# grailbio/bigslice

Measured on AMD Instinct MI355X. Metric: rows/sec (whole node) Reshuffle+Reduce group-by, higher is better.
Workload: dtype int64; 1 GPU; model=Reshuffle+Reduce group-by-sum (BASELINE config 3), rows_total=125000000, rows_per_gpu=125000000, distinct_keys=1000000, global_batch=125000000, parallelism=dp1, device=cuda:0

## Files before the change

bigslice_amd/csrc/ext.hip:

```cpp

#include <torch/extension.h>

#include <ATen/hip/HIPContext.h>
#include <hip/hip_runtime.h>

#include <vector>

#include "hash_partition.hip"
#include "groupby.hip"
#include "groupby_part.hip"
#include "sort.hip"
#include "radix.hip"
#include "runs.hip"
#include "runs_multi.hip"
#include "vecagg.hip"
#include "strings.hip"
#include "expr.hip"
#include "tokenize.hip"
#include "groupby_multi.hip"
#include "iddict.hip"
#include "bytes_gather.hip"

namespace {

#define HIP_CHECK(expr)                                              \
  do {                                                               \
    hipError_t _e = (expr);                                          \
    TORCH_CHECK(_e == hipSuccess, "HIP error: ",                     \
                hipGetErrorString(_e));                              \
  } while (0)

int32_t dtype_code(const torch::Tensor& t) {
  switch (t.scalar_type()) {
    case torch::kInt8: return DT_I8;
    case torch::kUInt8: return DT_U8;
    case torch::kInt16: return DT_I16;
    case torch::kInt32: return DT_I32;
    case torch::kInt64: return DT_I64;
    case torch::kFloat32: return DT_F32;
    case torch::kFloat64: return DT_F64;
    case torch::kBool: return DT_BOOL;
    case torch::kUInt32: return DT_U32;
    case torch::kUInt64: return DT_U64;
    default:
      TORCH_CHECK(false, "unsupported column dtype ", t.scalar_type());
  }
}

KeyCols make_key_cols(const std::vector<torch::Tensor>& cols) {
  TORCH_CHECK(!cols.empty() && (int)cols.size() <= MAX_KEY_COLS,
              "1..", MAX_KEY_COLS, " key columns supported");
  KeyCols k;
  k.n = (int)cols.size();
  for (size_t i = 0; i < cols.size(); ++i) {
    TORCH_CHECK(cols[i].is_cuda() && cols[i].is_contiguous(),
                "key columns must be contiguous device tensors");
    k.cols[i] = {cols[i].data_ptr(), dtype_code(cols[i])};
  }
  return k;
}

hipStream_t current_stream() {
  return at::hip::getCurrentHIPStream().stream();
}

int grid_blocks(int64_t n, int threads = THREADS) {
  return (int)std::min<int64_t>((n + threads - 1) / threads, 32768);
}

#define LAUNCH_NK(kernel, nk, blocks, threads, ...)                       \
  do {                                                                    \
    switch (nk) {                                                         \
      case 2:                                                             \
        hipLaunchKernelGGL(kernel<2>, dim3(blocks), dim3(threads), 0,     \
                           current_stream(), __VA_ARGS__);                \
        break;                                                            \
      case 3:                                                             \
        hipLaunchKernelGGL(kernel<3>, dim3(blocks), dim3(threads), 0,     \
                           current_stream(), __VA_ARGS__);                \
        break;                                                            \
      case 4:                                                             \
        hipLaunchKernelGGL(kernel<4>, dim3(blocks), dim3(threads), 0,     \
                           current_stream(), __VA_ARGS__);                \
        break;                                                            \
      default:                                                            \
        hipLaunchKernelGGL(kernel<0>, dim3(blocks), dim3(threads), 0,     \
                           current_stream(), __VA_ARGS__);                \
    }                                                                     \
    HIP_CHECK(hipGetLastError());                                         \
  } while (0)

int64_t int64_cols(const std::vector<torch::Tensor>& cols, int lo, int hi,
                   const char* what) {
// ... 351 lines not shown
  HIP_CHECK(hipGetLastError());
  return clean;
}

void groupby_insert_part(torch::Tensor keys, torch::Tensor vals,
                         torch::Tensor tkeys, torch::Tensor tab,
                         torch::Tensor flags, int64_t max_probes,
                         int64_t nbuckets, int64_t owned,
                         int64_t group_tiles) {
  TORCH_CHECK(keys.is_cuda() && keys.scalar_type() == torch::kInt64);
  TORCH_CHECK(vals.scalar_type() == torch::kInt64 &&
              vals.size(0) == keys.size(0));
  TORCH_CHECK(tab.scalar_type() == torch::kInt64);
  keys = keys.contiguous();
  vals = vals.contiguous();
  if (keys.size(0) == 0) return;
  int64_t cap = table_cap(tkeys, {tab}, flags);
  auto parts = part_scatter_impl(keys, vals, cap, nbuckets, group_tiles);
  const torch::Tensor& pairs = std::get<0>(parts);
  if (owned)
    part_owned_impl(pairs, std::get<1>(parts), tkeys, tab, flags,
                    max_probes);
  else
    launch_gbp_aggregate(pairs, tkeys, tab, flags, cap, max_probes);
}

std::tuple<torch::Tensor, torch::Tensor> groupby_part_scatter(
    torch::Tensor keys, torch::Tensor vals, int64_t cap,
    int64_t nbuckets, int64_t group_tiles) {
  TORCH_CHECK(keys.is_cuda() && keys.scalar_type() == torch::kInt64);
  TORCH_CHECK(vals.scalar_type() == torch::kInt64 &&
              vals.size(0) == keys.size(0));
  return part_scatter_impl(keys.contiguous(), vals.contiguous(), cap,
                           nbuckets, group_tiles);
}

void groupby_part_aggregate(torch::Tensor pairs, torch::Tensor tkeys,
                            torch::Tensor tab, torch::Tensor flags,
                            int64_t max_probes) {
  TORCH_CHECK(pairs.is_cuda() && pairs.scalar_type() == torch::kInt64 &&
              pairs.is_contiguous() && pairs.dim() == 2 &&
              pairs.size(1) == 2);
  if (pairs.size(0) == 0) return;
  TORCH_CHECK(tab.scalar_type() == torch::kInt64);
  launch_gbp_aggregate(pairs, tkeys, tab, flags,
                       table_cap(tkeys, {tab}, flags), max_probes);
}

torch::Tensor groupby_part_owned(torch::Tensor pairs, torch::Tensor totals,
                                 torch::Tensor tkeys, torch::Tensor tab,
                                 torch::Tensor flags, int64_t max_probes) {
  TORCH_CHECK(pairs.is_cuda() && pairs.scalar_type() == torch::kInt64 &&
              pairs.is_contiguous() && pairs.dim() == 2 &&
              pairs.size(1) == 2);
  TORCH_CHECK(totals.is_cuda() && totals.scalar_type() == torch::kInt32 &&
              totals.is_contiguous() && totals.dim() == 1);
  TORCH_CHECK(tab.scalar_type() == torch::kInt64);
  return part_owned_impl(pairs, totals, tkeys, tab, flags, max_probes);
}

std::vector<torch::Tensor> groupby_compact(torch::Tensor tkeys,
                                           std::vector<torch::Tensor> tabs,
                                           torch::Tensor cursor) {
  int64_t cap = tkeys.size(0) - 1;
  CompactCols cc;
  cc.n = (int)tabs.size();
  std::vector<torch::Tensor> out;
  auto out_keys = torch::empty({cap}, tkeys.options());
  out.push_back(out_keys);
  for (size_t c = 0; c < tabs.size(); ++c) {
    out.push_back(torch::empty({cap}, tabs[c].options()));
    cc.tab[c] = {tabs[c].data_ptr(), dtype_code(tabs[c])};
    cc.out[c] = {out[c + 1].data_ptr(), dtype_code(tabs[c])};
  }
  int64_t spb = (cap + 2047) / 2048;
  if (spb < THREADS) spb = THREADS;
  int blocks = (int)((cap + spb - 1) / spb);
  hipLaunchKernelGGL(k_groupby_compact, dim3(blocks), dim3(THREADS), 0,
                     current_stream(), tkeys.data_ptr<int64_t>(), cap, spb,
                     cc, out_keys.data_ptr<int64_t>(),
                     (unsigned long long*)cursor.data_ptr());
  HIP_CHECK(hipGetLastError());
  return out;
}


uint64_t gbm_fp_mask(int64_t fp_bits) {
  TORCH_CHECK(fp_bits >= 1 && fp_bits <= 64, "fp_bits must be in [1, 64]");
  return fp_bits == 64 ? ~uint64_t(0) : (uint64_t(1) << fp_bits) - 1;
}

int64_t gbm_batch_keys(MkCols& kc, const std::vector<torch::Tensor>& keys) {
  const int64_t n = int64_cols(keys, 2, MAX_KEY_COLS, "key columns");
  kc.n = (int)keys.size();
  for (size_t c = 0; c < keys.size(); ++c) {
    kc.src[c] = keys[c].data_ptr<int64_t>();
    kc.tab[c] = nullptr;
  }
  return n;
}

int64_t gbm_table(MkCols& kc, const torch::Tensor& tags,
                  const std::vector<torch::Tensor>& kcols,
                  at::ArrayRef<torch::Tensor> tabs,
                  const torch::Tensor& flags) {
  const int64_t cap = table_cap(tags, tabs, flags);
  TORCH_CHECK(cap <= (int64_t(1) << 31), "capacity above 2^31");
  TORCH_CHECK(flags.numel() >= 3, "flags must be int32[3]");
  TORCH_CHECK((int)kcols.size() == kc.n, "one key array per key column");
  for (size_t c = 0; c < kcols.size(); ++c) {
    TORCH_CHECK(kcols[c].is_cuda() && kcols[c].is_contiguous() &&
                kcols[c].scalar_type() == torch::kInt64 &&
                kcols[c].dim() == 1 && kcols[c].size(0) == cap + 1);
    kc.tab[c] = kcols[c].data_ptr<int64_t>();
  }
  return cap;
}

torch::Tensor groupby_mk_fingerprint(std::vector<torch::Tensor> keys,
                                     int64_t fp_bits) {
  MkCols kc{};
  const int64_t n = gbm_batch_keys(kc, keys);
  const uint64_t fp_mask = gbm_fp_mask(fp_bits);
  auto out = torch::empty({n}, keys[0].options());
  if (n == 0) return out;
  LAUNCH_NK(k_gbm_fingerprint, kc.n, grid_blocks(n), THREADS, kc, n,
            GB_HASH_SEED, fp_mask, out.data_ptr<int64_t>());
  return out;
}

torch::Tensor groupby_mk_claim(std::vector<torch::Tensor> keys,
                               torch::Tensor tags,
                               std::vector<torch::Tensor> kcols,
                               torch::Tensor flags, int64_t max_probes,
                               int64_t fp_bits) {
  MkCols kc{};
  const int64_t n = gbm_batch_keys(kc, keys);
  const int64_t cap = gbm_table(kc, tags, kcols, {}, flags);
  const uint64_t fp_mask = gbm_fp_mask(fp_bits);
  TORCH_CHECK(max_probes >= 1);
  auto slots = torch::empty({n}, keys[0].options().dtype(torch::kInt32));
  if (n == 0) return slots;
  LAUNCH_NK(k_gbm_claim, kc.n, grid_blocks(n), THREADS, kc, n,
            tags.data_ptr<int64_t>(), cap, GB_HASH_SEED, fp_mask,
            (uint32_t*)slots.data_ptr<int32_t>(),
            flags.data_ptr<int32_t>() + 1, max_probes);
  return slots;
}

void groupby_mk_accum(std::vector<torch::Tensor> keys,
                      std::vector<torch::Tensor> vals,
                      std::vector<int64_t> aggs, torch::Tensor slots,
                      torch::Tensor tags, std::vector<torch::Tensor> kcols,
                      std::vector<torch::Tensor> tabs,
                      torch::Tensor flags) {
  MkCols kc{};
  const int64_t n = gbm_batch_keys(kc, keys);
  const int64_t cap = gbm_table(kc, tags, kcols, tabs, flags);
  TORCH_CHECK(keys.size() + vals.size() <= (size_t)MAX_COLS,
              "at most ", MAX_COLS, " key and value columns");
  TORCH_CHECK(slots.is_cuda() && slots.is_contiguous() &&
              slots.scalar_type() == torch::kInt32 && slots.dim() == 1 &&
              slots.size(0) == n);
  ValCols vc = make_val_cols(vals, tabs, aggs);
  for (const auto& v : vals)
    TORCH_CHECK(v.dim() == 1 && v.size(0) == n,
// ... 737 lines not shown
                     overflow.data_ptr<int32_t>(), max_probes);
  HIP_CHECK(hipGetLastError());
}


std::vector<torch::Tensor> bytes_gather(torch::Tensor data,
                                        torch::Tensor offsets,
                                        torch::Tensor rows, int64_t total) {
  TORCH_CHECK(data.is_cuda() && data.is_contiguous() && data.dim() == 1 &&
                  data.scalar_type() == torch::kUInt8,
              "bytes_gather: contiguous uint8 device data required");
  TORCH_CHECK(offsets.is_cuda() && offsets.is_contiguous() &&
                  offsets.dim() == 1 && offsets.size(0) >= 1 &&
                  offsets.scalar_type() == torch::kInt64,
              "bytes_gather: contiguous int64 device offsets required");
  TORCH_CHECK(rows.is_cuda() && rows.dim() == 1 &&
                  rows.scalar_type() == torch::kInt64,
              "bytes_gather: int64 device row indices required");
  rows = rows.contiguous();
  const int64_t n = offsets.size(0) - 1;
  const int64_t m = rows.size(0);
  auto out_offsets = torch::zeros({m + 1}, offsets.options());
  if (m == 0 || total == 0)
    return {torch::empty({0}, data.options()), out_offsets};
  auto stream = current_stream();
  auto lens = torch::empty({m}, offsets.options());
  hipLaunchKernelGGL(k_bg_lens, dim3(grid_blocks(m)), dim3(THREADS), 0,
                     stream, offsets.data_ptr<int64_t>(), n,
                     rows.data_ptr<int64_t>(), m, lens.data_ptr<int64_t>());
  HIP_CHECK(hipGetLastError());
  auto incl = out_offsets.narrow(0, 1, m);
  at::cumsum_out(incl, lens, 0);
  if (total < 0) total = out_offsets[m].item<int64_t>();
  if (total == 0) return {torch::empty({0}, data.options()), out_offsets};
  auto out_data = torch::empty({total}, data.options());
  TORCH_CHECK(((uintptr_t)out_data.data_ptr<uint8_t>() & 15) == 0,
              "bytes_gather: output must be 16-byte aligned");
  const int64_t ntiles = (total + BG_TILE - 1) / BG_TILE;
  TORCH_CHECK(ntiles < (int64_t(1) << 31), "bytes_gather: result too large");
  hipLaunchKernelGGL(k_bg_copy, dim3((uint32_t)ntiles), dim3(BG_BLOCK), 0,
                     stream, data.data_ptr<uint8_t>(), data.size(0),
                     offsets.data_ptr<int64_t>(), n,
                     rows.data_ptr<int64_t>(), m,
                     out_offsets.data_ptr<int64_t>(), total,
                     out_data.data_ptr<uint8_t>());
  HIP_CHECK(hipGetLastError());
  return {out_data, out_offsets};
}

}

PYBIND11_MODULE(TORCH_EXTENSION_NAME, m) {
  m.def("hash_columns", &hash_columns, "murmur3 row hash (K3)");
  m.def("hash_partition", &hash_partition,
        "fused hash+histogram+scatter partitioner (K4)");
  m.def("scatter_by_partition", &scatter_by_partition,
        "scatter rows by precomputed partition ids");
  m.def("groupby_insert", &groupby_insert,
        "hash-aggregate insert pass (K9)");
  m.def("groupby_insert_lds", &groupby_insert_lds,
        "two-level LDS+global insert (int64 sum)");
  m.def("groupby_insert_part", &groupby_insert_part,
        "partitioned LDS pre-aggregating insert (single i64 sum)",
        py::arg("keys"), py::arg("vals"), py::arg("tkeys"), py::arg("tab"),
        py::arg("flags"), py::arg("max_probes"), py::arg("nbuckets"),
        py::arg("owned") = 0, py::arg("group_tiles") = 0);
  m.def("groupby_part_owned", &groupby_part_owned,
        "owner + cleanup passes of the partitioned insert; returns clean");
  m.attr("GBP_OWN_LIMIT") = (int64_t)GBP_OWN_LIMIT;
  m.def("groupby_part_scatter", &groupby_part_scatter,
        "bucket scatter of the partitioned insert", py::arg("keys"),
        py::arg("vals"), py::arg("cap"), py::arg("nbuckets"),
        py::arg("group_tiles") = 0);
  m.def("groupby_part_group_tiles", &part_group_tiles,
        "tiles per group the partitioned insert picks for n rows");
  m.attr("GBP_SCATTER_ROWS") = (int64_t)GBP_SCATTER_ROWS;
  m.def("groupby_part_aggregate", &groupby_part_aggregate,
        "aggregate pass of the partitioned insert");
  m.attr("GBP_TILE_ROWS") = (int64_t)GBP_TILE_ROWS;
  m.attr("GBP_LDS_SLOTS") = (int64_t)GBP_LDS_SLOTS;
  m.attr("GBP_MAX_BUCKETS") = (int64_t)GBP_MAX_BUCKETS;
  m.def("groupby_compact", &groupby_compact,
        "hash-aggregate table compaction (K9)");
  m.def("groupby_mk_insert", &groupby_mk_insert,
        "multi-column-key hash-aggregate insert: claim + accumulate (K21)",
        py::arg("keys"), py::arg("vals"), py::arg("aggs"), py::arg("tags"),
        py::arg("kcols"), py::arg("tabs"), py::arg("flags"),
        py::arg("max_probes"), py::arg("fp_bits") = 64);
  m.def("groupby_mk_claim", &groupby_mk_claim,
        "launch 1 of groupby_mk_insert; returns the rows' slots");
  m.def("groupby_mk_accum", &groupby_mk_accum,
        "launch 2 of groupby_mk_insert");
  m.def("groupby_mk_fingerprint", &groupby_mk_fingerprint,
        "the tuple fingerprint groupby_mk_insert claims slots by",
        py::arg("keys"), py::arg("fp_bits") = 64);
  m.attr("MAX_KEY_COLS") = (int64_t)MAX_KEY_COLS;
  m.attr("MAX_COLS") = (int64_t)MAX_COLS;
  m.def("agg_identity", &agg_identity, "aggregation identity fill");
  m.def("radix_argsort", &radix_argsort, "device radix argsort (K6)");
  m.def("radix_sort_keys", &radix_sort_keys, "device radix key sort",
        py::arg("keys"), py::arg("probe") = true);
  m.def("runs_sorted", &runs_sorted,
        "run boundaries of sorted keys (K18)");
  m.def("runs_multi", &runs_multi,
        "run boundaries of lexicographically sorted key columns (K22)");
  m.attr("MRUNS_TILE_ROWS") = (int64_t)MRUNS_TILE;
  m.def("lex_searchsorted", &lex_searchsorted,
        "searchsorted over lexicographically sorted tuples (K22)",
        py::arg("sorted_cols"), py::arg("query_cols"),
        py::arg("right") = false);
  m.def("segment_reduce_runs", &segment_reduce_runs,
        "int64 segmented reduce with precomputed runs (K16 fast path)");
  m.def("runs_guard", &runs_guard,
        "(count, max run length) of a runs_sorted result");
  m.def("segment_reduce_sorted", &segment_reduce_sorted,
        "typed reduce-by-key over sorted pairs (K16; deterministic)");
  m.def("hash_bytes", &hash_bytes,
        "murmur3-32 over varlen byte rows (K17, device strings)");
  m.def("hash_bytes64", &hash_bytes64,
        "64-bit two-seed murmur3 dictionary ids (K17)");
  m.def("colsum16", &colsum16,
        "vector-aggregate experiment: [N,16] f32 colsum, VALU vs MFMA");
  m.def("radix_sort_kv", &radix_sort_kv,
        "direct (key, 8-byte value) radix sort");
  m.def("slot_pids", &slot_pids, "table-slot-range partition ids");
  m.def("expr_apply", &expr_apply,
        "fused Map/Filter expression interpreter (K13)");
  m.def("tokenize_bytes", &tokenize_bytes,
        "split BYTES rows into tokens on a delimiter set (K20)");
  m.attr("TOKENIZE_TILE_BYTES") = (int64_t)TOK_TILE;
  m.def("iddict_claim", &iddict_claim,
        "id dictionary: claim slots for new ids; returns the new rows (K23)");
  m.def("iddict_lookup", &iddict_lookup,
        "id dictionary: position of every id, -1 when absent (K23)");
  m.def("iddict_rehash", &iddict_rehash,
        "id dictionary: move a table into a larger one (K23)");
  m.def("bytes_gather", &bytes_gather,
        "variable-length row gather of a BYTES column (K23)",
        py::arg("data"), py::arg("offsets"), py::arg("rows"),
        py::arg("total") = -1);
  m.attr("BYTES_GATHER_TILE_BYTES") = (int64_t)BG_TILE;
}
```

bigslice_amd/csrc/groupby.hip:

```cpp

#include <hip/hip_runtime.h>

#include "hashtable.h"

#define THREADS 256

struct CompactCols {
  ColDesc tab[MAX_COLS];
  MutColDesc out[MAX_COLS];
  int n;
};

__device__ __forceinline__ void copy_elt(const MutColDesc& dst, int64_t di,
                                         const ColDesc& src, int64_t si) {
  switch (elt_size(src.code)) {
    case 1: ((uint8_t*)dst.ptr)[di] = ((const uint8_t*)src.ptr)[si]; break;
    case 2: ((uint16_t*)dst.ptr)[di] = ((const uint16_t*)src.ptr)[si]; break;
    case 4: ((uint32_t*)dst.ptr)[di] = ((const uint32_t*)src.ptr)[si]; break;
    default: ((uint64_t*)dst.ptr)[di] = ((const uint64_t*)src.ptr)[si];
  }
}

extern "C" __global__ void k_groupby_compact(
    const int64_t* tkeys, int64_t cap, int64_t slots_per_block,
// ... 58 lines not shown
    if (cur == GB_SENTINEL) {
      long long prev = atomicCAS((unsigned long long*)&lk[h],
                                 (unsigned long long)GB_SENTINEL,
                                 (unsigned long long)k);
      cur = (prev == GB_SENTINEL) ? k : prev;
    }
    if (cur == k) {
      atomicAdd((unsigned long long*)&lv[h], (unsigned long long)v);
      return true;
    }
    h = (h + 1) & (GB_LDS_SLOTS - 1);
  }
  return false;
}

extern "C" __global__ void k_groupby_insert_sum_i64_lds(
    const int64_t* keys, const int64_t* vals, int64_t n, int64_t* tkeys,
    long long* tab, int64_t cap, uint32_t seed, int32_t* sentinel_seen,
    int32_t* overflow, int64_t max_probes) {
  __shared__ long long lk[GB_LDS_SLOTS];
  __shared__ long long lv[GB_LDS_SLOTS];
  for (int i = threadIdx.x; i < GB_LDS_SLOTS; i += blockDim.x) {
    lk[i] = GB_SENTINEL;
    lv[i] = 0;
  }
  __syncthreads();
  uint64_t gmask = (uint64_t)cap - 1;
  int64_t stride = (int64_t)gridDim.x * blockDim.x;
  int64_t i = (int64_t)blockIdx.x * blockDim.x + threadIdx.x;
  for (; i < n; i += stride) {
    int64_t k = keys[i];
    long long v = (long long)vals[i];
    if (k == GB_SENTINEL || !gb_lds_try(k, v, lk, lv, seed))
      gb_global_insert_sum(k, v, tkeys, tab, gmask, cap, seed,
                           sentinel_seen, overflow, max_probes);
  }
  __syncthreads();
  for (int i2 = threadIdx.x; i2 < GB_LDS_SLOTS; i2 += blockDim.x) {
    if (lk[i2] != GB_SENTINEL)
      gb_global_insert_sum(lk[i2], lv[i2], tkeys, tab, gmask, cap, seed,
                           sentinel_seen, overflow, max_probes);
  }
}

extern "C" __global__ void k_slot_pids(const int64_t* keys, int64_t n,
                                       int64_t cap, int32_t nparts,
                                       uint32_t seed, int32_t* pids) {
  int64_t i = (int64_t)blockIdx.x * blockDim.x + threadIdx.x;
  int64_t stride = (int64_t)gridDim.x * blockDim.x;
  uint64_t mask = (uint64_t)cap - 1;
  uint64_t shift = 0;
  while (((uint64_t)cap >> shift) > (uint64_t)nparts) ++shift;
  for (; i < n; i += stride) {
    uint64_t h = mm3_u64((uint64_t)keys[i], seed) & mask;
    pids[i] = (int32_t)(h >> shift);
  }
}

extern "C" __global__ void k_groupby_insert(
    const int64_t* keys, int64_t n, ValCols vals, int64_t* tkeys,
    int64_t cap, uint32_t seed, int32_t* sentinel_seen, int32_t* overflow,
    int64_t max_probes) {
  int64_t i = (int64_t)blockIdx.x * blockDim.x + threadIdx.x;
  int64_t stride = (int64_t)gridDim.x * blockDim.x;
  uint64_t mask = (uint64_t)cap - 1;
  for (; i < n; i += stride) {
    int64_t k = keys[i];
    int64_t slot;
    if (k == GB_SENTINEL) {
      if (atomicOr(sentinel_seen, 1) == 0) {}
      slot = cap;
    } else {
      uint64_t h = mm3_u64((uint64_t)k, seed) & mask;
      if (gb_probe_claim(tkeys, h, mask, k, max_probes) == GB_FULL) {
        atomicOr(overflow, 1);
        return;
      }
      slot = (int64_t)h;
    }
    for (int c = 0; c < vals.n; ++c)
      accum(vals.tab[c], slot, vals.src[c], i, vals.agg[c]);
  }
}
```

bigslice_amd/kernels/groupby.py:

```python

from __future__ import annotations

import dataclasses
import math
import os
import sys
from typing import List, Optional

import torch

from .. import kernels as _k
from . import _C, native
from .sortedkeys import sort_combine

_AGG_CODES = {"sum": 0, "min": 1, "max": 2, "prod": 3}

_GB_KEY_DTYPES = (torch.int64,)
_GB_VAL_DTYPES = (torch.int64, torch.int32, torch.float32, torch.float64)

GB_SENTINEL = -(1 << 63)
MAX_PROBES = 128

PART_TILE_ROWS = _C.GBP_TILE_ROWS if _C is not None else None
PART_LDS_SLOTS = _C.GBP_LDS_SLOTS if _C is not None else None
PART_MAX_BUCKETS = _C.GBP_MAX_BUCKETS if _C is not None else None

PART_OWN_LIMIT = _C.GBP_OWN_LIMIT if _C is not None else None


@dataclasses.dataclass(frozen=True)
class Options:
    mode: Optional[str] = None
    combine: str = "auto"
    part: bool = True
    part_owned: bool = True
    part_group: int = 0
    lds_blocks: int = 4096
    sample_rows: int = 1 << 19
    debug: bool = False

    @classmethod
    def from_env(cls, env=None) -> "Options":
        env = os.environ if env is None else env
        mode = env.get("BIGSLICE_GB_MODE")
        return cls(
            mode=mode if mode in ("lds", "global", "part") else None,
            combine=env.get("BIGSLICE_GB_COMBINE", "auto"),
            part=env.get("BIGSLICE_GB_PART", "1") == "1",
            part_owned=env.get("BIGSLICE_GB_PART_OWNED", "1") == "1",
            part_group=int(env.get("BIGSLICE_GB_PART_GROUP", "0")),
            lds_blocks=int(env.get("BIGSLICE_GB_LDS_BLOCKS", "4096")),
            sample_rows=int(env.get("BIGSLICE_GB_SAMPLE_ROWS",
                                    str(1 << 19))),
            debug=bool(env.get("BIGSLICE_GB_DEBUG")))


def _next_pow2(n: int, floor: int = 1024) -> int:
    c = floor
    while c < n:
        c <<= 1
    return c


def first_capacity(cap_hint: Optional[int], n: int, floor: int = 1024) -> int:
    from .. import config
    return _next_pow2(cap_hint or min(
        2 * n, getattr(config, "GROUPBY_INITIAL_CAP", 1 << 23)), floor)


def part_buckets(n: int, nkeys: float, cap: int,
                 lds_slots: int = PART_LDS_SLOTS,
                 tile_rows: int = PART_TILE_ROWS,
                 max_buckets: int = PART_MAX_BUCKETS) -> int:
    room = lds_slots / 2 - tile_rows * nkeys / max(n, 1)
    b = 2
    while b < max_buckets and (room <= 0 or b * room < nkeys):
        b <<= 1
    return min(b, cap)


def part_owned_buckets(n: int, cap: int, lds_slots: int, tile_rows: int,
                       max_buckets: int):
    want = max(cap / lds_slots, n / tile_rows)
    b = 2
    while b < want:
        b <<= 1
    b = max(2, min(b, max_buckets, cap))
    s = cap // b
    return (b, s) if s <= lds_slots else None


PART_BAND = (6.0, 500.0)


def forced_mode(opts: Options, sum_i64: bool) -> Optional[str]:
    if opts.mode in ("lds", "global"):
        return opts.mode
    if opts.mode == "part" and not sum_i64:
        return "global"
    if opts.combine == "sort":
        return "sort"
    return None


def choose_mode(distinct: int, sample_n: int, batch_n: int, sum_i64: bool,
                opts: Options, cap_hint: Optional[int] = None):
    forced = forced_mode(opts, sum_i64)
    if forced:
        return forced, None, cap_hint
    s = sample_n
    K = None
    if distinct < s:
        K = float(distinct)
        for _ in range(20):
            K = distinct / (1.0 - math.exp(-s / K))
        if cap_hint is None:
            cap_hint = _next_pow2(min(max(int(4 * K), 1024), 1 << 30))
    if distinct * 32 <= s:
        mode = "lds"
    elif distinct * 100 > s * 88:
        mode = "sort"
    else:
        rows_per_key = batch_n / max(K, 1.0)
        mode = "sort" if rows_per_key > 500 else "global"
        if (mode == "global" and sum_i64 and opts.part
                and PART_BAND[0] <= rows_per_key <= PART_BAND[1]):
            mode = "part"
    if opts.mode == "part":
        mode = "part"
    elif mode == "sort" and opts.combine == "hash":
        mode = "global"
    return mode, K, cap_hint


def part_plan(n: int, cap: int, key_estimate: Optional[float],
              opts: Options, lds_slots: int, tile_rows: int,
# ... 4 lines not shown
                             max_buckets) if opts.part_owned else None
    if own is not None:
        return "owned", own[0]
    nkeys = key_estimate or cap / 4
    return "tiled", part_buckets(n, nkeys, cap, lds_slots, tile_rows,
                                 max_buckets)


def regrow_capacity(cap: int, rows: int) -> int:
    new = cap
    while new < 4 * rows and new < (1 << 30):
        new <<= 1
    if new == cap:
        new <<= 1
    if new > (1 << 31):
        raise RuntimeError("groupby table overflow")
    return new


def groupby_supported(keys: torch.Tensor, vals: List[torch.Tensor],
                      aggs: List[str]) -> bool:
    return (native(keys.is_cuda, "groupby") and groupby_shape_supported(
        [keys.dtype], [v.dtype for v in vals], aggs))


def groupby_shape_supported(key_dtypes, val_dtypes, aggs) -> bool:
    return (all(dt in _GB_KEY_DTYPES for dt in key_dtypes)
            and all(dt in _GB_VAL_DTYPES for dt in val_dtypes)
            and all(isinstance(a, str) and a in _AGG_CODES for a in aggs))


class HashTable:

    def _ensure_alloc(self, n: int):
        if self.cap is None:
            self._alloc(first_capacity(self.cap_hint, n))

    def _agg_arrays(self, cap: int) -> List:
        return [
            _k._C.agg_identity(torch.empty(0, dtype=dt, device=self.device),
                            code, cap + 1)
            for dt, code in zip(self.val_dtypes, self.codes)]

    def _compact(self):
        cursor = torch.zeros(1, dtype=torch.int64, device=self.device)
        outs = _k._C.groupby_compact(*self._slots(), cursor)
        host = torch.cat([cursor, self.flags.to(torch.int64)]).cpu()
        return outs, host.tolist()

    def _regrow(self):
        batches = self.batches
        self._alloc(regrow_capacity(self.cap, self.rows))
        self.batches = []
        for keys, vals in batches:
            self._insert_now(keys, vals)


class GroupTable(HashTable):

    _SMALL_BATCH = 1 << 21
    _PART_MIN_ROWS = 1 << 21

    def __init__(self, val_dtypes, aggs: List[str], device,
                 cap_hint: int = None):
        self.opts = Options.from_env()
        self.aggs = aggs
        self.codes = [_AGG_CODES[a] for a in aggs]
        self.device = device
        self.val_dtypes = list(val_dtypes)
        self.cap = None
        self.cap_hint = cap_hint
        self.tkeys = None
        self.tabs: List = []
        self.flags = None
        self.batches: List = []
        self._deferred: List = []
        self.rows = 0
        self._mode: Optional[str] = None
        self._sample_forced: Optional[str] = None
        self._sample_n = 0
        self._sample_batch_n = 0
        self._sample_ne = None
        self._key_estimate: Optional[float] = None

    @property
    def _sum_i64(self) -> bool:
        return (len(self.val_dtypes) == 1
                and self.val_dtypes[0] == torch.int64
                and self.aggs == ["sum"])

    def _alloc(self, cap: int):
        self.cap = cap
        dev = self.device
        self.tkeys = torch.full((cap + 1,), GB_SENTINEL,
                                dtype=torch.int64, device=dev)
        self.tabs = self._agg_arrays(cap)
        self.flags = torch.zeros(2, dtype=torch.int32, device=dev)

    def _slots(self):
        return self.tkeys, self.tabs

    @property
    def _sort_combinable(self) -> bool:
        return (_k._C is not None
                and str(self.device).startswith("cuda")
                and all(a in ("sum", "min", "max") for a in self.aggs)
                and all(dt in _GB_VAL_DTYPES for dt in self.val_dtypes))

    def _start_sample(self, keys: torch.Tensor) -> None:
        self._sample_forced = forced_mode(self.opts, self._sum_i64)
        if self._sample_forced:
            return
        prefix = min(keys.shape[0], self.opts.sample_rows)
        sk = _k._C.radix_sort_keys(keys[:prefix].contiguous(),
                                probe=False)
        self._sample_n = prefix
        self._sample_batch_n = keys.shape[0]
        self._sample_ne = (sk[1:] != sk[:-1]).sum()

    def _read_sample(self) -> str:
        if self._sample_forced:
            return self._sample_forced
        distinct = 1 + int(self._sample_ne.item())
        mode, self._key_estimate, self.cap_hint = choose_mode(
            distinct, self._sample_n, self._sample_batch_n, self._sum_i64,
            self.opts, self.cap_hint)
        if self.opts.debug:
            print(f"[gb] sample={self._sample_n} distinct={distinct} "
                  f"cap_hint={self.cap_hint} mode={mode}",
                  file=sys.stderr, flush=True)
        return mode

    def insert(self, keys: torch.Tensor, vals: List[torch.Tensor]):
        n = keys.shape[0]
        if n == 0:
            return
        self.rows += n
        if not self._sort_combinable:
            self._insert_now(keys, vals)
            return
        if self._mode is None:
            if n >= self._SMALL_BATCH:
                self._start_sample(keys)
                self._mode = "pending"
            self._deferred.append((keys, vals))
            return
        if self._mode == "pending":
            self._mode = self._read_sample()
        if self._mode == "sort":
            self._deferred.append((keys, vals))
            return
        self._flush_deferred()
        self._insert_now(keys, vals)

    def _flush_deferred(self):
        pending, self._deferred = self._deferred, []
        for k, v in pending:
            self._insert_now(k, v)

    def _insert_now(self, keys: torch.Tensor, vals: List[torch.Tensor]):
        self._ensure_alloc(keys.shape[0])
        self.batches.append((keys, vals))
        mode = self._mode if self._sum_i64 else None
        plan = part_plan(
            keys.shape[0], self.cap, self._key_estimate, self.opts,
            PART_LDS_SLOTS, PART_TILE_ROWS, PART_MAX_BUCKETS,
            self._PART_MIN_ROWS) if mode == "part" else None
        if mode == "lds":
            _k._C.groupby_insert_lds(keys, vals[0], self.tkeys, self.tabs[0],
                                  self.flags, MAX_PROBES,
                                  self.opts.lds_blocks)
        elif plan is not None:
            kind, nbuckets = plan
            _k._C.groupby_insert_part(keys, vals[0], self.tkeys, self.tabs[0],
                                   self.flags, MAX_PROBES, nbuckets,
                                   1 if kind == "owned" else 0,
                                   self.opts.part_group)
        else:
            _k._C.groupby_insert(keys, list(vals), self.codes, self.tkeys,
                              self.tabs, self.flags, MAX_PROBES)

    def _finish_deferred(self):
        from ..utils import stats
        if self._mode not in (None, "sort"):
            self._flush_deferred()
            return None
        batches = self._deferred
        keys = (batches[0][0] if len(batches) == 1
                else torch.cat([k for k, _ in batches]))
        if self._mode is None:
            self._start_sample(keys)
            self._mode = self._read_sample()
            if self._mode != "sort":
                self._flush_deferred()
                return None
        self._deferred = []
        vcols = (list(batches[0][1]) if len(batches) == 1
                 else [torch.cat(cols)
                       for cols in zip(*(v for _, v in batches))])
        uk, outs = sort_combine(keys, vcols, self.codes)
        if self.cap is not None:
            self._insert_now(uk, outs)
            return None
        stats.DEFAULT.add("combiner/keys", int(uk.shape[0]))
        return uk, outs

    def finish(self):
        from ..utils import stats
        stats.DEFAULT.add("combiner/records", self.rows)
        if self._mode == "pending":
            self._mode = self._read_sample()
        if self._deferred:
            done = self._finish_deferred()
            if done is not None:
                return done
        if self.cap is None:
            empty = torch.empty(0, dtype=torch.int64, device=self.device)
            return empty, [torch.empty(0, dtype=dt, device=self.device)
                           for dt in self.val_dtypes]
        while True:
            outs, (nkeys, sentinel_seen, overflow) = self._compact()
            if overflow:
                self._regrow()
                continue
            keys = outs[0][:nkeys]
            vals = [o[:nkeys] for o in outs[1:]]
            if sentinel_seen:
                keys = torch.cat([keys, torch.full(
                    (1,), GB_SENTINEL, dtype=torch.int64,
                    device=self.device)])
                vals = [torch.cat([v, t[self.cap:self.cap + 1]])
                        for v, t in zip(vals, self.tabs)]
            self.batches = []
            stats.DEFAULT.add("combiner/keys", int(keys.shape[0]))
            return keys, vals


def groupby(keys: torch.Tensor, vals: List[torch.Tensor],
            aggs: List[str]):
    t = GroupTable([v.dtype for v in vals], aggs, keys.device)
    t.insert(keys, list(vals))
    return t.finish()
```

bigslice_amd/ops/aggregate.py:

```python

from __future__ import annotations

import functools
import operator
import os
from typing import Callable, List, Optional, Sequence, Union

import torch

from .. import config
from ..frame import Frame
from ..schema import Schema, is_object

BUILTIN_AGGS = ("sum", "min", "max", "prod")

_CALLABLE_MAP = {
    operator.add: "sum",
    operator.mul: "prod",
    min: "min",
    max: "max",
}


def resolve_agg(fn: Union[str, Callable]) -> Union[str, Callable]:
# ... 188 lines not shown

    def result_frames(self, chunk: int):
        for f in self.inner.result_frames(chunk):
            pos = torch.searchsorted(
                self.dict_ids, f.columns[0].to(self.dict_ids.device))
            keys = self.dict_keys.select(pos)
            yield Frame([keys] + list(f.columns[1:]), 1,
                        combined_id=f.combined_id)


class TensorAggregator:

    def __init__(self, schema: Schema, agg: Aggregation, device: str):
        self.schema = schema
        self.nkey = schema.prefix
        self.agg = agg
        self.device = device
        self.keys: Optional[List[torch.Tensor]] = None
        self.vals: List[torch.Tensor] = []
        self._pending = _Pending()
        self._pt_frames: Optional[List[Frame]] = []
        self._pt_id = None
        self._table = None
        if device.startswith("cuda"):
            from .. import kernels
            from ..kernels import groupby_multi as gbm
            if self.nkey == 1:
                supported = kernels.groupby_shape_supported
                make = kernels.GroupTable
            else:
                def supported(*shape):
                    return (gbm.multikey_supported(*shape)
                            and gbm.Options.from_env().enabled)
                make = functools.partial(
                    gbm.MultiKeyTable, self.nkey,
                    fallback=lambda k, v: _combine_once(k, v, self.agg))
            val_dts = schema.dtypes[self.nkey:]
            if supported(schema.dtypes[:self.nkey], val_dts, agg.aggs) \
                    and kernels.native(True, "groupby"):
                self._table = make(val_dts, agg.aggs, device)

    def add(self, frame: Frame) -> None:
        if len(frame) == 0:
            return
        if frame.device != self.device:
            frame = frame.to(self.device)
        if self._pt_frames is not None:
            cid = frame.combined_id
            if cid is not None and (self._pt_id is None
                                    or cid == self._pt_id):
                self._pt_id = cid
                self._pt_frames.append(frame)
                return
            buffered, self._pt_frames = self._pt_frames, None
            for f in buffered:
                self._add_normal(f)
        self._add_normal(frame)

    def _add_normal(self, frame: Frame) -> None:
        if self._table is not None:
            self._pending.feed(frame, self._table_insert)
            return
        self._pending.add(frame)
        if self._pending.rows >= config.COMBINER_TARGET_KEYS:
            self._flush()

    def _table_insert(self, f: Frame) -> None:
        vals = [c.contiguous() for c in f.columns[self.nkey:]]
        if self.nkey == 1:
            self._table.insert(f.columns[0].contiguous(), vals)
        else:
            self._table.insert(list(f.columns[:self.nkey]), vals)

    def _flush(self) -> None:
        f = self._pending.take()
        if f is None:
            return
        keys = [c for c in f.columns[: self.nkey]]
        vals = list(f.columns[self.nkey:])
        if self.keys is not None:
            keys = [torch.cat([sk, k]) for sk, k in zip(self.keys, keys)]
            vals = [torch.cat([sv, v]) for sv, v in zip(self.vals, vals)]
        self.keys, self.vals = _combine_once(keys, vals, self.agg)

    def result_frames(self, chunk: int):
        if self._pt_frames is not None:
            for f in self._pt_frames:
                yield f
            return
        if self._table is not None:
            self._pending.flush(self._table_insert)
            keys, vals = self._table.finish()
            keys = [keys] if self.nkey == 1 else keys
            if keys[0].shape[0]:
                self.keys, self.vals = keys, vals
        else:
            self._flush()
        if self.keys is None:
            return
        import uuid
        cid = uuid.uuid4().int & ((1 << 63) - 1)
        n = self.keys[0].shape[0]
        for off in range(0, n, chunk):
            stop = min(off + chunk, n)
            yield Frame([k[off:stop] for k in self.keys] +
                        [v[off:stop] for v in self.vals],
                        self.schema.prefix, combined_id=cid)


def _combine_once(keys: List[torch.Tensor], vals: List[torch.Tensor],
                  agg: Aggregation):
    from ..kernels.groupby import _AGG_CODES
    from ..kernels.sortedkeys import _SCATTER_OP
    if len(keys) == 1:
        k = keys[0]
        if k.is_cuda:
            from .. import kernels
            if kernels.groupby_supported(k, vals, agg.aggs):
                uk, ov = kernels.groupby(k, vals, agg.aggs)
                return [uk], ov
        uk, inv = torch.unique(k, return_inverse=True)
        nseg = uk.shape[0]
        uks = [uk]
    else:
        n = keys[0].shape[0]
        perm = torch.arange(n, device=keys[0].device)
        for kc in reversed(keys):
            _, o = torch.sort(kc[perm], stable=True)
            perm = perm[o]
        skeys = [kc[perm] for kc in keys]
        boundary = torch.zeros(n, dtype=torch.bool,
                               device=keys[0].device)
        boundary[0] = True
        for kc in skeys:
            boundary[1:] |= kc[1:] != kc[:-1]
        inv_sorted = boundary.cumsum(0) - 1
        nseg = int(inv_sorted[-1].item()) + 1 if n else 0
        uks = [kc[boundary] for kc in skeys]
        inv = torch.empty(n, dtype=torch.int64, device=keys[0].device)
        inv[perm] = inv_sorted
        vals = list(vals)
    out_vals = []
    for v, a in zip(vals, agg.aggs):
        init = torch.empty(nseg, dtype=v.dtype, device=v.device)
        out = init.scatter_reduce_(
            0, inv, v, reduce=_SCATTER_OP[_AGG_CODES[a]], include_self=False)
        out_vals.append(out)
    return uks, out_vals


class DictAggregator:

    def __init__(self, schema: Schema, agg: Aggregation):
        self.schema = schema
        self.agg = agg
        self.state = {}

    def add(self, frame: Frame) -> None:
        nkey = self.schema.prefix
        lists = frame.column_lists()
        keys = list(zip(*lists[:nkey])) if nkey > 1 else lists[0]
        vals = lists[nkey:]
        state = self.state
        aggs = self.agg.aggs
        if len(vals) == 1 and aggs == ["sum"]:
            vcol = vals[0]
# ... 53 lines not shown
```

bigslice_amd/runtime/partition.py:

```python

from __future__ import annotations

from typing import Callable, List, Optional

import torch

from ..frame import Frame


def partition_ids(frame: Frame, num_partitions: int,
                  partitioner: Optional[Callable] = None) -> torch.Tensor:
    if partitioner is not None:
        p = partitioner(frame, num_partitions)
        if not isinstance(p, torch.Tensor):
            p = torch.tensor(list(p), dtype=torch.int64)
        return p.to(torch.int64)
    h = frame.hash(0)
    return (h.to(torch.int64) & 0xFFFFFFFF) % num_partitions


def split_frame(frame: Frame, num_partitions: int,
                partitioner: Optional[Callable] = None) -> List[Optional[Frame]]:
    if num_partitions == 1:
        return [frame]
    if len(frame) == 0:
        return [None] * num_partitions
    if frame.device != "cpu" and not frame.has_objects:
        from .. import kernels
        if num_partitions <= 4096 and kernels.partition_supported(frame):
            return kernels.partition_frame(frame, num_partitions,
                                           partitioner)
    p = partition_ids(frame, num_partitions, partitioner)
    order = torch.argsort(p, stable=True)
    sorted_f = frame.select(order)
    counts = torch.bincount(p, minlength=num_partitions)
    out: List[Optional[Frame]] = []
    off = 0
    for c in counts.tolist():
        out.append(sorted_f.slice(off, off + c) if c else None)
        off += c
    return out


class SharedPhaseCombiner:

    def __init__(self, schema, combiner, device: str, num_partitions: int,
                 expected_tasks: int, chunk: int):
        import threading

        from ..ops.aggregate import make_aggregator
        self.agg = make_aggregator(schema, combiner, device)
        self.device = device
        self.num_partitions = num_partitions
        self.chunk = chunk
        self.remaining = expected_tasks
        self.lock = threading.Lock()
        self.events = []
        self.rows = 0

    def add(self, frame: Frame) -> None:
        with self.lock:
            self.rows += len(frame)
            self.agg.add(frame)

    def task_done(self) -> bool:
        if self.device.startswith("cuda"):
            ev = torch.cuda.Event()
            ev.record()
        else:
            ev = None
        with self.lock:
            if ev is not None:
                self.events.append(ev)
            self.remaining -= 1
            return self.remaining == 0

    def finish_buckets(self) -> List[List[Frame]]:
        if self.device.startswith("cuda"):
            cur = torch.cuda.current_stream()
            for ev in self.events:
                cur.wait_event(ev)
        buckets: List[List[Frame]] = \
            [[] for _ in range(self.num_partitions)]
        for f in self.agg.result_frames(self.chunk * 4):
            for pi, pf in enumerate(split_frame(f, self.num_partitions,
                                                None)):
                if pf is not None and len(pf):
                    buckets[pi].append(pf)
        return buckets


class PartitionWriter:

    def __init__(self, num_partitions: int, partitioner, combiner,
                 schema, device: str, chunk: int):
        self.num_partitions = num_partitions
        self.partitioner = partitioner
        self.schema = schema
        self.device = device
        self.chunk = chunk
        self.rows = 0
        self.agg = None
        self.aggs = None
        self.buckets: List[List[Frame]] = \
            [[] for _ in range(num_partitions)]
        if combiner is not None:
            from ..ops.aggregate import make_aggregator
            if partitioner is None:
                self.agg = make_aggregator(schema, combiner, device)
            else:
                self.aggs = [make_aggregator(schema, combiner, device)
                             for _ in range(num_partitions)]

    def add(self, frame: Frame) -> None:
        self.rows += len(frame)
        if self.agg is not None:
            self.agg.add(frame)
            return
        parts = split_frame(frame, self.num_partitions, self.partitioner)
        from ..frame import over_high_water
        tier = frame.device != "cpu" and over_high_water()
        for pi, pf in enumerate(parts):
            if pf is None or len(pf) == 0:
                continue
            if self.aggs is not None:
                self.aggs[pi].add(pf)
            elif tier:
                self.buckets[pi].append(pf.to_pinned_host())
            else:
                self.buckets[pi].append(pf)

    def finish(self) -> List[List[Frame]]:
        if self.agg is not None:
            for f in self.agg.result_frames(self.chunk * 4):
                parts = split_frame(f, self.num_partitions, None)
                for pi, pf in enumerate(parts):
                    if pf is not None and len(pf):
                        self.buckets[pi].append(pf)
            return self.buckets
        if self.aggs is not None:
            return [list(a.result_frames(self.chunk)) for a in self.aggs]
        return self.buckets
```

Measured before the change: 29.14 billion rows/sec.

## Compact group-by table directly into hash partitions and hash-sample distinct keys

Adds a three-kernel finish (count, offsets, write) that compacts the hash-aggregate table straight into per-partition contiguous output, so the separate compact followed by split_frame per chunk is no longer needed. It also replaces the sort-based distinct-key sample estimate with a hash-table claim count on the device. Both paths are enabled by default and fall back to the old route when conditions are not met. The cost is an extra histogram pass over the table, plus a host sync for the partition counts.

```diff
diff --git a/bigslice_amd/csrc/ext.hip b/bigslice_amd/csrc/ext.hip
--- a/bigslice_amd/csrc/ext.hip
+++ b/bigslice_amd/csrc/ext.hip
@@ -9,6 +9,7 @@
 #include "hash_partition.hip"
 #include "groupby.hip"
 #include "groupby_part.hip"
+#include "groupby_finish.hip"
 #include "sort.hip"
 #include "radix.hip"
 #include "runs.hip"
@@ -526,6 +527,88 @@
                      (unsigned long long*)cursor.data_ptr());
   HIP_CHECK(hipGetLastError());
   return out;
+}
+
+std::pair<int64_t, int64_t> gbf_blocks(int64_t cap, int64_t nparts) {
+  int64_t blocks = std::min<int64_t>(
+      GBF_THREADS, std::max<int64_t>(64, (int64_t(1) << 18) / nparts));
+  blocks = std::min(blocks, (cap + 1 + 2047) / 2048);
+  int64_t spb = (cap + 1 + blocks - 1) / blocks;
+  spb += spb & 1;
+  return {(cap + 1 + spb - 1) / spb, spb};
+}
+
+std::tuple<std::vector<torch::Tensor>, torch::Tensor>
+groupby_compact_partition(torch::Tensor tkeys,
+                          std::vector<torch::Tensor> tabs,
+                          torch::Tensor flags, int64_t nparts) {
+  TORCH_CHECK(nparts >= 1 && nparts <= MAX_LDS_PARTS &&
+                  nparts <= GBF_MAX_PARTS,
+              "nparts must be in [1, ", MAX_LDS_PARTS, "]");
+  const int64_t cap = table_cap(tkeys, tabs, flags);
+  TORCH_CHECK(cap <= (int64_t(1) << 31), "capacity above 2^31");
+  FinishCols fc;
+  fc.n = (int)tabs.size();
+  TORCH_CHECK(fc.n <= MAX_COLS, "at most ", MAX_COLS, " value columns");
+  std::vector<torch::Tensor> out;
+  out.push_back(torch::empty({cap + 1}, tkeys.options()));
+  for (int c = 0; c < fc.n; ++c) {
+    const auto st = tabs[c].scalar_type();
+    TORCH_CHECK(st == torch::kInt64 || st == torch::kInt32 ||
+                    st == torch::kFloat32 || st == torch::kFloat64,
+                "unsupported value dtype ", st);
+    out.push_back(torch::empty({cap + 1}, tabs[c].options()));
+    fc.tab[c] = {tabs[c].data_ptr(), dtype_code(tabs[c])};
+    fc.out[c] = {out[c + 1].data_ptr(), dtype_code(tabs[c])};
+  }
+  const auto [blocks, spb] = gbf_blocks(cap, nparts);
+  auto opts32 = tkeys.options().dtype(torch::kInt32);
+  auto hist = torch::empty({nparts * blocks}, opts32);
+  auto totals = torch::empty({nparts}, opts32);
+  auto dev = torch::empty({nparts + 2}, tkeys.options());
+  auto stream = current_stream();
+  const uint32_t np = (uint32_t)nparts;
+  const int32_t* fl = flags.data_ptr<int32_t>();
+  hipLaunchKernelGGL(k_gbf_count, dim3((uint32_t)blocks), dim3(GBF_THREADS),
+                     0, stream, tkeys.data_ptr<int64_t>(), cap, spb, np, fl,
+                     (uint32_t*)hist.data_ptr<int32_t>());
+  HIP_CHECK(hipGetLastError());
+  hipLaunchKernelGGL(k_gbf_offsets, dim3(np), dim3(GBF_THREADS), 0, stream,
+                     (uint32_t*)hist.data_ptr<int32_t>(), (uint32_t)blocks,
+                     np, fl, (uint32_t*)totals.data_ptr<int32_t>(),
+                     dev.data_ptr<int64_t>());
+  HIP_CHECK(hipGetLastError());
+  hipLaunchKernelGGL(k_gbf_write, dim3((uint32_t)blocks), dim3(GBF_THREADS),
+                     0, stream, tkeys.data_ptr<int64_t>(), cap, spb, np, fl,
+                     (const uint32_t*)hist.data_ptr<int32_t>(),
+                     (const uint32_t*)totals.data_ptr<int32_t>(), fc,
+                     out[0].data_ptr<int64_t>());
+  HIP_CHECK(hipGetLastError());
+  return {out, dev.cpu()};
+}
+
+torch::Tensor groupby_sample_distinct(torch::Tensor keys, int64_t rows) {
+  TORCH_CHECK(keys.is_cuda() && keys.scalar_type() == torch::kInt64 &&
+              keys.dim() == 1 && keys.stride(0) == 1);
+  TORCH_CHECK(rows >= 1 && rows <= keys.size(0) &&
+                  rows <= (int64_t(1) << 30),
+              "1 <= rows <= min(len(keys), 2^30)");
+  int64_t m = 2;
+  while (m < 2 * rows) m <<= 1;
+  auto tags = torch::empty({m}, keys.options());
+  auto state = torch::empty({2}, keys.options());
+  auto result = state.select(0, 0);
+  auto stream = current_stream();
+  hipLaunchKernelGGL(k_gbs_init, dim3(grid_blocks(m / 2)), dim3(THREADS), 0,
+                     stream, tags.data_ptr<int64_t>(), m,
+                     state.data_ptr<int64_t>());
+  HIP_CHECK(hipGetLastError());
+  hipLaunchKernelGGL(k_gbs_count, dim3(grid_blocks((rows + 1) / 2)),
+                     dim3(THREADS), 0, stream, keys.data_ptr<int64_t>(),
+                     rows, tags.data_ptr<int64_t>(), m,
+                     state.data_ptr<int64_t>());
+  HIP_CHECK(hipGetLastError());
+  return result;
 }
 
 
@@ -1429,6 +1512,11 @@
   m.attr("GBP_MAX_BUCKETS") = (int64_t)GBP_MAX_BUCKETS;
   m.def("groupby_compact", &groupby_compact,
         "hash-aggregate table compaction (K9)");
+  m.def("groupby_compact_partition", &groupby_compact_partition,
+        "compact a group-by table straight into hash partitions");
+  m.attr("MAX_LDS_PARTS") = (int64_t)MAX_LDS_PARTS;
+  m.def("groupby_sample_distinct", &groupby_sample_distinct,
+        "distinct keys of a prefix, minus one, as a device scalar");
   m.def("groupby_mk_insert", &groupby_mk_insert,
         "multi-column-key hash-aggregate insert: claim + accumulate (K21)",
         py::arg("keys"), py::arg("vals"), py::arg("aggs"), py::arg("tags"),
diff --git a/bigslice_amd/csrc/groupby.hip b/bigslice_amd/csrc/groupby.hip
--- a/bigslice_amd/csrc/groupby.hip
+++ b/bigslice_amd/csrc/groupby.hip
@@ -164,3 +164,67 @@
       accum(vals.tab[c], slot, vals.src[c], i, vals.agg[c]);
   }
 }
+
+extern "C" __global__ void k_gbs_init(int64_t* tags, int64_t m,
+                                      int64_t* state) {
+  const int64_t stride = (int64_t)gridDim.x * blockDim.x;
+  int64_t i = (int64_t)blockIdx.x * blockDim.x + threadIdx.x;
+  if (i == 0) {
+    state[0] = -1;
+    state[1] = 0;
+  }
+  const longlong2 empty = {GB_SENTINEL, GB_SENTINEL};
+  for (; 2 * i < m; i += stride) *(longlong2*)(tags + 2 * i) = empty;
+}
+
+__device__ __forceinline__ uint32_t gbs_claim(int64_t k, int64_t* tags,
+                                              uint64_t mask, int32_t* flag) {
+  if (k == GB_SENTINEL)
+    return *(volatile int32_t*)flag == 0 && atomicOr(flag, 1) == 0;
+  uint64_t h = gbm_fmix64((uint64_t)k) & mask;
+  return gb_probe_claim(tags, h, mask, k, (int64_t)mask + 1) == GB_CLAIMED;
+}
+
+template <bool WIDE>
+__device__ __forceinline__ uint32_t gbs_count_rows(const int64_t* keys,
+                                                   int64_t rows,
+                                                   int64_t* tags,
+                                                   uint64_t mask,
+                                                   int32_t* flag) {
+  const int64_t stride = (int64_t)gridDim.x * blockDim.x;
+  int64_t t = (int64_t)blockIdx.x * blockDim.x + threadIdx.x;
+  uint32_t mine = 0;
+  if constexpr (WIDE) {
+    for (int64_t i = 2 * t; i < rows; i += 2 * stride) {
+      if (i + 1 < rows) {
+        const longlong2 two = *(const longlong2*)(keys + i);
+        mine += gbs_claim(two.x, tags, mask, flag);
+        mine += gbs_claim(two.y, tags, mask, flag);
+      } else {
+        mine += gbs_claim(keys[i], tags, mask, flag);
+      }
+    }
+  } else {
+    for (int64_t i = t; i < rows; i += stride)
+      mine += gbs_claim(keys[i], tags, mask, flag);
+  }
+  return mine;
+}
+
+extern "C" __global__ __launch_bounds__(THREADS) void k_gbs_count(
+    const int64_t* keys, int64_t rows, int64_t* tags, int64_t m,
+    int64_t* state) {
+  __shared__ uint32_t claimed;
+  if (threadIdx.x == 0) claimed = 0;
+  __syncthreads();
+  const uint64_t mask = (uint64_t)m - 1;
+  int32_t* flag = (int32_t*)(state + 1);
+  const uint32_t mine =
+      ((uintptr_t)keys & 15) == 0
+          ? gbs_count_rows<true>(keys, rows, tags, mask, flag)
+          : gbs_count_rows<false>(keys, rows, tags, mask, flag);
+  if (mine) atomicAdd(&claimed, mine);
+  __syncthreads();
+  if (threadIdx.x == 0 && claimed)
+    atomicAdd((unsigned long long*)state, (unsigned long long)claimed);
+}
diff --git a/bigslice_amd/csrc/groupby_finish.hip b/bigslice_amd/csrc/groupby_finish.hip
--- /dev/null
+++ b/bigslice_amd/csrc/groupby_finish.hip
@@ -0,0 +1,156 @@
+
+#include <hip/hip_runtime.h>
+
+#include "hashtable.h"
+
+#define GBF_THREADS 512
+#define GBF_WAVES (GBF_THREADS / 64)
+#define GBF_MAX_PARTS 4096
+#define GBF_SCAN_C (GBF_MAX_PARTS / GBF_THREADS)
+
+struct FinishCols {
+  ColDesc tab[MAX_COLS];
+  MutColDesc out[MAX_COLS];
+  int n;
+};
+
+__device__ __forceinline__ uint32_t gbf_part(int64_t k, uint32_t nparts) {
+  return mm3_u64((uint64_t)k, 0u) % nparts;
+}
+
+template <bool WIDE, typename F>
+__device__ __forceinline__ void gbf_live_slots(const int64_t* tkeys,
+                                               int64_t cap, bool sentinel,
+                                               int64_t start, int64_t end,
+                                               F f) {
+  auto one = [&](int64_t i, int64_t k) {
+    if (i < cap ? k != GB_SENTINEL : sentinel) f(i, k);
+  };
+  if constexpr (WIDE) {
+    for (int64_t i = start + 2 * threadIdx.x; i < end;
+         i += 2 * GBF_THREADS) {
+      if (i + 1 < end) {
+        const longlong2 two = *(const longlong2*)(tkeys + i);
+        one(i, two.x);
+        one(i + 1, two.y);
+      } else {
+        one(i, tkeys[i]);
+      }
+    }
+  } else {
+    for (int64_t i = start + threadIdx.x; i < end; i += GBF_THREADS)
+      one(i, tkeys[i]);
+  }
+}
+
+extern "C" __global__ __launch_bounds__(GBF_THREADS) void k_gbf_count(
+    const int64_t* tkeys, int64_t cap, int64_t slots_per_block,
+    uint32_t nparts, const int32_t* flags, uint32_t* hist) {
+  __shared__ uint32_t lh[GBF_MAX_PARTS];
+  for (uint32_t p = threadIdx.x; p < nparts; p += GBF_THREADS) lh[p] = 0;
+  __syncthreads();
+  const int64_t start = (int64_t)blockIdx.x * slots_per_block;
+  const int64_t end = min(start + slots_per_block, cap + 1);
+  const bool sentinel = flags[0] != 0;
+  auto count = [&](int64_t, int64_t k) {
+    atomicAdd(&lh[gbf_part(k, nparts)], 1u);
+  };
+  if (((uintptr_t)tkeys & 15) == 0)
+    gbf_live_slots<true>(tkeys, cap, sentinel, start, end, count);
+  else
+    gbf_live_slots<false>(tkeys, cap, sentinel, start, end, count);
+  __syncthreads();
+  for (uint32_t p = threadIdx.x; p < nparts; p += GBF_THREADS)
+    hist[(int64_t)p * gridDim.x + blockIdx.x] = lh[p];
+}
+
+__device__ __forceinline__ uint32_t gbf_block_scan(uint32_t x,
+                                                   uint32_t* wtmp,
+                                                   uint32_t* total) {
+  const int lane = threadIdx.x & 63;
+  const int w = threadIdx.x >> 6;
+  uint32_t run = x;
+  for (int off = 1; off < 64; off <<= 1) {
+    const uint32_t up = __shfl_up(run, off);
+    if (lane >= off) run += up;
+  }
+  if (lane == 63) wtmp[w] = run;
+  __syncthreads();
+  uint32_t base = 0, all = 0;
+  for (int w2 = 0; w2 < GBF_WAVES; ++w2) {
+    if (w2 < w) base += wtmp[w2];
+    all += wtmp[w2];
+  }
+  *total = all;
+  __syncthreads();
+  return base + run - x;
+}
+
+extern "C" __global__ __launch_bounds__(GBF_THREADS) void k_gbf_offsets(
+    uint32_t* hist, uint32_t nblocks, uint32_t nparts, const int32_t* flags,
+    uint32_t* totals, int64_t* host) {
+  __shared__ uint32_t wtmp[GBF_WAVES];
+  const uint32_t p = blockIdx.x;
+  uint32_t* row = hist + (int64_t)p * nblocks;
+  const bool ok = threadIdx.x < nblocks;
+  const uint32_t x = ok ? row[threadIdx.x] : 0;
+  uint32_t total;
+  const uint32_t excl = gbf_block_scan(x, wtmp, &total);
+  if (ok) row[threadIdx.x] = excl;
+  if (threadIdx.x == 0) {
+    totals[p] = total;
+    host[p] = (int64_t)total;
+    if (p == 0) {
+      host[nparts] = flags[0];
+      host[nparts + 1] = flags[1];
+    }
+  }
+}
+
+__device__ __forceinline__ void gbf_copy_elt(const MutColDesc& dst,
+                                             int64_t di, const ColDesc& src,
+                                             int64_t si) {
+  if (elt_size(src.code) == 4)
+    ((uint32_t*)dst.ptr)[di] = ((const uint32_t*)src.ptr)[si];
+  else
+    ((uint64_t*)dst.ptr)[di] = ((const uint64_t*)src.ptr)[si];
+}
+
+extern "C" __global__ __launch_bounds__(GBF_THREADS) void k_gbf_write(
+    const int64_t* tkeys, int64_t cap, int64_t slots_per_block,
+    uint32_t nparts, const int32_t* flags, const uint32_t* hist,
+    const uint32_t* totals, FinishCols cols, int64_t* out_keys) {
+  __shared__ uint32_t lcur[GBF_MAX_PARTS];
+  __shared__ uint32_t wtmp[GBF_WAVES];
+  uint32_t t[GBF_SCAN_C];
+  uint32_t sum = 0;
+#pragma unroll
+  for (int j = 0; j < GBF_SCAN_C; ++j) {
+    const uint32_t p = threadIdx.x * GBF_SCAN_C + j;
+    t[j] = p < nparts ? totals[p] : 0;
+    sum += t[j];
+  }
+  uint32_t unused;
+  uint32_t run = gbf_block_scan(sum, wtmp, &unused);
+#pragma unroll
+  for (int j = 0; j < GBF_SCAN_C; ++j) {
+    const uint32_t p = threadIdx.x * GBF_SCAN_C + j;
+    if (p < nparts)
+      lcur[p] = run + hist[(int64_t)p * gridDim.x + blockIdx.x];
+    run += t[j];
+  }
+  __syncthreads();
+  const int64_t start = (int64_t)blockIdx.x * slots_per_block;
+  const int64_t end = min(start + slots_per_block, cap + 1);
+  const bool sentinel = flags[0] != 0;
+  auto put = [&](int64_t i, int64_t k) {
+    const int64_t pos = atomicAdd(&lcur[gbf_part(k, nparts)], 1u);
+    out_keys[pos] = k;
+    for (int c = 0; c < cols.n; ++c)
+      gbf_copy_elt(cols.out[c], pos, cols.tab[c], i);
+  };
+  if (((uintptr_t)tkeys & 15) == 0)
+    gbf_live_slots<true>(tkeys, cap, sentinel, start, end, put);
+  else
+    gbf_live_slots<false>(tkeys, cap, sentinel, start, end, put);
+}
diff --git a/bigslice_amd/kernels/groupby.py b/bigslice_amd/kernels/groupby.py
--- a/bigslice_amd/kernels/groupby.py
+++ b/bigslice_amd/kernels/groupby.py
@@ -37,6 +37,8 @@
     part_group: int = 0
     lds_blocks: int = 4096
     sample_rows: int = 1 << 19
+    sample: str = "hash"
+    finish_part: bool = True
     debug: bool = False
 
     @classmethod
@@ -52,6 +54,9 @@
             lds_blocks=int(env.get("BIGSLICE_GB_LDS_BLOCKS", "4096")),
             sample_rows=int(env.get("BIGSLICE_GB_SAMPLE_ROWS",
                                     str(1 << 19))),
+            sample=("sort" if env.get("BIGSLICE_GB_SAMPLE") == "sort"
+                    else "hash"),
+            finish_part=env.get("BIGSLICE_GB_FINISH_PART", "1") == "1",
             debug=bool(env.get("BIGSLICE_GB_DEBUG")))
 
 
@@ -222,6 +227,8 @@
         self._sample_batch_n = 0
         self._sample_ne = None
         self._key_estimate: Optional[float] = None
+        self._settled = False
+        self._done = None
 
     @property
     def _sum_i64(self) -> bool:
@@ -252,10 +259,14 @@
         if self._sample_forced:
             return
         prefix = min(keys.shape[0], self.opts.sample_rows)
+        self._sample_n = prefix
+        self._sample_batch_n = keys.shape[0]
+        if self.opts.sample == "hash" and native(keys.is_cuda, "groupby"):
+            self._sample_ne = _k._C.groupby_sample_distinct(
+                keys.contiguous(), prefix)
+            return
         sk = _k._C.radix_sort_keys(keys[:prefix].contiguous(),
                                 probe=False)
-        self._sample_n = prefix
-        self._sample_batch_n = keys.shape[0]
         self._sample_ne = (sk[1:] != sk[:-1]).sum()
 
     def _read_sample(self) -> str:
@@ -345,19 +356,51 @@
         stats.DEFAULT.add("combiner/keys", int(uk.shape[0]))
         return uk, outs
 
-    def finish(self):
+    def _settle(self):
         from ..utils import stats
+        if self._settled:
+            return self._done
+        self._settled = True
         stats.DEFAULT.add("combiner/records", self.rows)
         if self._mode == "pending":
             self._mode = self._read_sample()
         if self._deferred:
-            done = self._finish_deferred()
-            if done is not None:
-                return done
-        if self.cap is None:
+            self._done = self._finish_deferred()
+        if self._done is None and self.cap is None:
             empty = torch.empty(0, dtype=torch.int64, device=self.device)
-            return empty, [torch.empty(0, dtype=dt, device=self.device)
-                           for dt in self.val_dtypes]
+            self._done = empty, [
+                torch.empty(0, dtype=dt, device=self.device)
+                for dt in self.val_dtypes]
+        return self._done
+
+    def finish_partitioned(self, nparts: int):
+        from ..utils import stats
+        if not (self.opts.finish_part
+                and 1 <= nparts <= _k._C.MAX_LDS_PARTS):
+            return None
+        if self._settle() is not None:
+            return None
+        while True:
+            outs, host = _k._C.groupby_compact_partition(
+                self.tkeys, self.tabs, self.flags, nparts)
+            *counts, _, overflow = host.tolist()
+            if overflow:
+                self._regrow()
+                continue
+            self.batches = []
+            stats.DEFAULT.add("combiner/keys", sum(counts))
+            parts, off = [], 0
+            for c in counts:
+                parts.append((outs[0][off:off + c],
+                              [o[off:off + c] for o in outs[1:]]))
+                off += c
+            return parts
+
+    def finish(self):
+        from ..utils import stats
+        done = self._settle()
+        if done is not None:
+            return done
         while True:
             outs, (nkeys, sentinel_seen, overflow) = self._compact()
             if overflow:
diff --git a/bigslice_amd/ops/aggregate.py b/bigslice_amd/ops/aggregate.py
--- a/bigslice_amd/ops/aggregate.py
+++ b/bigslice_amd/ops/aggregate.py
@@ -294,6 +294,22 @@
             keys = [torch.cat([sk, k]) for sk, k in zip(self.keys, keys)]
             vals = [torch.cat([sv, v]) for sv, v in zip(self.vals, vals)]
         self.keys, self.vals = _combine_once(keys, vals, self.agg)
+
+    def result_partitions(self, nparts: int, chunk: int):
+        if (self._pt_frames is not None or self._table is None
+                or self.nkey != 1 or not self.device.startswith("cuda")):
+            return None
+        self._pending.flush(self._table_insert)
+        parts = self._table.finish_partitioned(nparts)
+        if parts is None:
+            return None
+        import uuid
+        cid = uuid.uuid4().int & ((1 << 63) - 1)
+        return [[Frame([keys[off:off + chunk]] +
+                       [v[off:off + chunk] for v in vals],
+                       self.schema.prefix, combined_id=cid)
+                 for off in range(0, keys.shape[0], chunk)]
+                for keys, vals in parts]
 
     def result_frames(self, chunk: int):
         if self._pt_frames is not None:
diff --git a/bigslice_amd/runtime/partition.py b/bigslice_amd/runtime/partition.py
--- a/bigslice_amd/runtime/partition.py
+++ b/bigslice_amd/runtime/partition.py
@@ -42,6 +42,20 @@
     return out
 
 
+def combined_buckets(agg, num_partitions: int,
+                     chunk: int) -> List[List[Frame]]:
+    fused = getattr(agg, "result_partitions", None)
+    buckets = fused(num_partitions, chunk) if fused is not None else None
+    if buckets is not None:
+        return buckets
+    buckets = [[] for _ in range(num_partitions)]
+    for f in agg.result_frames(chunk):
+        for pi, pf in enumerate(split_frame(f, num_partitions, None)):
+            if pf is not None and len(pf):
+                buckets[pi].append(pf)
+    return buckets
+
+
 class SharedPhaseCombiner:
 
     def __init__(self, schema, combiner, device: str, num_partitions: int,
@@ -80,14 +94,8 @@
             cur = torch.cuda.current_stream()
             for ev in self.events:
                 cur.wait_event(ev)
-        buckets: List[List[Frame]] = \
-            [[] for _ in range(self.num_partitions)]
-        for f in self.agg.result_frames(self.chunk * 4):
-            for pi, pf in enumerate(split_frame(f, self.num_partitions,
-                                                None)):
-                if pf is not None and len(pf):
-                    buckets[pi].append(pf)
-        return buckets
+        return combined_buckets(self.agg, self.num_partitions,
+                                self.chunk * 4)
 
 
 class PartitionWriter:
@@ -132,12 +140,8 @@
 
     def finish(self) -> List[List[Frame]]:
         if self.agg is not None:
-            for f in self.agg.result_frames(self.chunk * 4):
-                parts = split_frame(f, self.num_partitions, None)
-                for pi, pf in enumerate(parts):
-                    if pf is not None and len(pf):
-                        self.buckets[pi].append(pf)
-            return self.buckets
+            return combined_buckets(self.agg, self.num_partitions,
+                                    self.chunk * 4)
         if self.aggs is not None:
             return [list(a.result_frames(self.chunk)) for a in self.aggs]
         return self.buckets
```

New measurement: 30.24 billion rows/sec (median of 6 runs). 1.04x the previous value.
